# osayamenja/FlashMoE

Hardware: AMD Instinct MI355X
Metric: DMoE fwd tokens/s (higher is better)
Workload: dtype bf16; 1 GPU; BASELINE configs[1]: 1xMI355X E=8 top-2 S=4096 H=1024 P=4096 bf16 (E=8N weak scaling at N ranks); seq_len=4096, d_model=1024, d_ff=4096, experts=8, top_k=2, capacity_factor=1, parallelism=ep1

## Files before the change

### flashmoe_amd/csrc/flashmoe_kernels.hip

```cpp

#include <hip/hip_runtime.h>
#include <hip/hip_bf16.h>
#include <hip/hip_fp16.h>

#include <cmath>
#include <cstdint>
#include <cstdio>
#include <cstring>
#include <algorithm>
#include <type_traits>

#include "../../include/flashmoe_abi.h"


using bf16 = __hip_bfloat16;

struct __align__(8) TPS {
  uint32_t tokenIdx;
  float probSum;
};
__device__ __host__ __forceinline__ uint32_t tpsTok(uint32_t v) {
  return v & 0x0FFFFFFFu;
}
__device__ __host__ __forceinline__ uint32_t tpsJ(uint32_t v) { return v >> 28; }
// ... 242 lines not shown
          if (!tk && lrow[e] > lv) { lv = lrow[e]; li = e; }
        }
#pragma unroll
        for (int off = 1; off < 8; off <<= 1) {
          if (off < SUBS) {
            const float ov = __shfl_xor(lv, off, SUBS);
            const int oi = __shfl_xor(li, off, SUBS);
            if (ov > lv || (ov == lv && oi < li)) { lv = ov; li = oi; }
          }
        }
        if (li >= e0 && li < e1) takenM |= 1ull << (li - e0);
        if (sub == 0) {
          sel[token * K + i] = (uint16_t)li;
          mCw += __expf(lv - m) * inv_d;
        }
      }
      if (sub == 0) sCw[token] = mCw;
    }
  }
  __syncthreads();
  for (int i = tid * 8; i < TT * PX; i += 512 * 8) {
    const int row = i / PX, col0 = i % PX;
    const float mR = sMax[row], ivR = sInv[row];
    const float* lrow = logits + row * (E + 1);
    struct __attribute__((aligned(16))) V8 { T x[8]; } v;
#pragma unroll
    for (int q = 0; q < 8; ++q) {
      const int col = col0 + q;
      const float pv = (col < E) ? __expf(lrow[col] - mR) * ivR : 0.0f;
      fromF(pv, v.x[q]);
    }
    *reinterpret_cast<V8*>(gate_out + (size_t)(pm0 + row) * PX + col0) = v;
  }
  __syncthreads();
  if (tid < E) {
    uint32_t cnt = 0;
    for (int mj = 0; mj < TT * K; mj += 8) {
      const u32x4 v = *reinterpret_cast<const u32x4*>(sel + mj);
#pragma unroll
      for (int q = 0; q < 8; ++q) {
        const uint32_t w = v[q >> 1];
        const uint16_t sv = (q & 1) ? (uint16_t)(w >> 16) : (uint16_t)(w & 0xffff);
        const bool mt = (sv == (uint16_t)tid);
        localIdx[mt ? (mj + q) : TT * K] = (uint16_t)cnt;
        cnt += mt;
      }
    }
    base[tid] = __hip_atomic_fetch_add(eC + tid, cnt, __ATOMIC_RELAXED,
                                       __HIP_MEMORY_SCOPE_AGENT);
    if (gML) {
      float colSum = 0.0f;
      for (int mj = 0; mj < TT; ++mj)
        colSum += __expf(logits[mj * (E + 1) + tid] - sMax[mj]) * sInv[mj];
      atomicAdd(gML + tid, colSum / (float)S);
      atomicAdd(gMeC + tid, (float)cnt / (float)S);
    }
  }
  __syncthreads();
  if (tid < TT) {
#pragma unroll
    for (int i = 0; i < K; ++i) {
      const int e = sel[tid * K + i];
      const uint32_t slot = base[e] + localIdx[tid * K + i];
      const bool keep = slot < (uint32_t)EC;
      if (keep) {
        tokenIds[(size_t)e * pEC + slot] =
            TPS{(uint32_t)(pm0 + tid) | ((uint32_t)i << 28), sCw[tid]};
      }
      if (kept) kept[(size_t)(pm0 + tid) * K + i] = keep ? 1 : 0;
    }
  }
  }
}

template <typename T, int K>
__global__ __launch_bounds__(512) void k_gate_route(
    float* __restrict__ logits32, T* __restrict__ gate_out,
    TPS* __restrict__ tokenIds, uint32_t* __restrict__ eC, int S, int E,
    int PX, int EC, int pEC, float* __restrict__ gML,
    float* __restrict__ gMeC, uint8_t* __restrict__ kept) {
  extern __shared__ __attribute__((aligned(16))) char smem[];
  route_tile_core<T, K>(smem, logits32, gate_out, tokenIds, eC, kept, gML,
                        gMeC, S, E, PX, EC, pEC, blockIdx.x * 128);
}


__device__ __forceinline__ uint32_t cvt2_fp8(float a, float b) {
  f32x2n v;
  v.x = a;
  v.y = b;
  return __builtin_amdgcn_cvt_pk_fp8_f32(v.x, v.y, 0u, false);
}

template <typename T>
__global__ void k_quant_mx(const T* __restrict__ in, uint8_t* __restrict__ out,
                           uint8_t* __restrict__ scales, long long nRows,
                           int K) {
  const int wave = (int)(threadIdx.x >> 6);
  const int lane = (int)(threadIdx.x & 63);
  const long long nBlk = nRows * (K / 64);
  for (long long b = (long long)blockIdx.x * 4 + wave; b < nBlk;
       b += (long long)gridDim.x * 4) {
    const long long row = b / (K / 64);
    const int j = (int)(b % (K / 64));
    const float v = toF(in[row * K + j * 64 + lane]);
    float m = fabsf(v);
#pragma unroll
    for (int off = 32; off > 0; off >>= 1)
      m = fmaxf(m, __shfl_xor(m, off, 64));
    int e = 0;
    if (m > 0.0f) {
      int ex;
      (void)frexpf(m / 448.0f, &ex);
      e = ex;
      if (e < -126) e = -126;
      if (e > 127) e = 127;
    }
    const float inv = exp2f((float)-e);
    const uint32_t pk = cvt2_fp8(v * inv, 0.0f);
    out[row * K + j * 64 + lane] = (uint8_t)(pk & 0xFF);
    if (lane == 0) scales[row * (K / 64) + j] = (uint8_t)(127 + e);
  }
}


struct GemmArgs {
  const void* A;
  const void* B;
  const void* bias;
  void* out;
  float* O32;
  void* moe_out;
  const void* gate_out;
  const TPS* tokenIds;
  const uint32_t* eC;
  long long strideAExpert;
  long long strideBExpert;
  long long strideOExpert;
  int K;
  int N;
  int EC, pEC, PX;
  int topk;
  int act;
  int expertOffset;
  int nRows;
  int H;
  int splitK;
  const int32_t* segExpert;
  int noRemap;
  int totalJobs;
  int jobsMT, jobsNT;
  int atomicLogits;
  int slotAlways;
  int sc1Out;
  const void* aScales;
  void* out8;
  void* outScales;
  long long gluOffset;
};

__device__ __forceinline__ float gate_act(float v, int act) {
  return act == 2 ? v / (1.0f + expf(-v))
                  : 0.5f * v * (1.0f + erff(v * 0.70710678118654752f));
}

typedef __attribute__((address_space(1))) const uint32_t gas_u32;
// ... 1676 lines not shown
      gemm_phase_walk<ET, 0, 256, 128, WET, 3, CH, CP>(
          gu, smem, f.upMT, f.upNT, f.upJobs, f.nBlocks, gu.act,
          gu.bias != nullptr, &f.ctl->upJobsDone, f.upRowDone,
          f.debugBits);
      break;
    default:
      gemm_phase_walk<ET, 0, 128, 128, WET, 2, CH, CP>(
          gu, smem, f.upMT, f.upNT, f.upJobs, f.nBlocks, gu.act,
          gu.bias != nullptr, &f.ctl->upJobsDone, f.upRowDone,
          f.debugBits);
      break;
  }
  if (tid == 0)
    atomicMax(reinterpret_cast<unsigned long long*>(&f.ctl->clk[2]),
              __builtin_amdgcn_s_memrealtime());

  switch (f.dnGeom) {
    case 0:
      gemm_phase_walk_dn<ET, 256, 256, WET, 2, CP, CH>(
          gd, f, smem, f.dnMT, f.dnNT, f.dnJobs, f.nBlocks,
          gd.bias != nullptr, &f.ctl->dnJobsDone);
      break;
    case 1:
      gemm_phase_walk_dn<ET, 128, 256, WET, 3, CP, CH>(
          gd, f, smem, f.dnMT, f.dnNT, f.dnJobs, f.nBlocks,
          gd.bias != nullptr, &f.ctl->dnJobsDone);
      break;
    case 3:
      gemm_phase_walk_dn<ET, 256, 128, WET, 3, CP, CH>(
          gd, f, smem, f.dnMT, f.dnNT, f.dnJobs, f.nBlocks,
          gd.bias != nullptr, &f.ctl->dnJobsDone);
      break;
    default:
      gemm_phase_walk_dn<ET, 128, 128, WET, 2, CP, CH>(
          gd, f, smem, f.dnMT, f.dnNT, f.dnJobs, f.nBlocks,
          gd.bias != nullptr, &f.ctl->dnJobsDone);
      break;
  }
  fused_wait(&f.ctl->dnJobsDone, (uint32_t)f.dnJobs, f.errWord,
             f.spinBound, (f.debugBits & 2) != 0);
  if (tid == 0)
    atomicMax(reinterpret_cast<unsigned long long*>(&f.ctl->clk[3]),
              __builtin_amdgcn_s_memrealtime());

  for (int j = blockIdx.x; j < f.cbJobs; j += f.nBlocks) {
    const int t0 = j * f.cbTB;
    const int t1 = min(f.S, t0 + f.cbTB);
    switch (f.topk) {
      case 1: combine_tokens<ET, 1>(f, t0, t1); break;
      case 2: combine_tokens<ET, 2>(f, t0, t1); break;
      case 3: combine_tokens<ET, 3>(f, t0, t1); break;
      case 4: combine_tokens<ET, 4>(f, t0, t1); break;
      case 5: combine_tokens<ET, 5>(f, t0, t1); break;
      case 6: combine_tokens<ET, 6>(f, t0, t1); break;
      case 7: combine_tokens<ET, 7>(f, t0, t1); break;
      default: combine_tokens<ET, 8>(f, t0, t1); break;
    }
  }
  if (tid == 0)
    atomicMax(reinterpret_cast<unsigned long long*>(&f.ctl->clk[4]),
              __builtin_amdgcn_s_memrealtime());
}


static int launch_group_gemm(hipStream_t st, int phase, const struct GemmArgs& a,
                             int M, int nE);

namespace {

struct State {
  fm_config cfg{};
  bool initialized = false;
  int rank = 0, world = 1;
  int S = 0, H = 0, P = 0, E = 0, PX = 0, nLx = 0, EC = 0, pEC = 0;
  size_t esz = 0;
  size_t wesz = 0;
  int wMats = 2;
  bool gated = false;
  TPS* tokenIds = nullptr;
  uint32_t* eC = nullptr;
  float* logits32 = nullptr;
  float* gML = nullptr;
  float* gMeC = nullptr;
  char* heap = nullptr;
  size_t heapRecvOff = 0, heapRetOff = 0, heapDFlagOff = 0, heapRFlagOff = 0;
  size_t heapBytes = 0;
  void* peerBase[64] = {};
  bool peerOpened[64] = {};
  uint64_t* dPeerRecv = nullptr;
  uint64_t* dPeerRet = nullptr;
  uint64_t* dPeerDFlag = nullptr;
  uint64_t* dPeerRFlag = nullptr;
  uint32_t* dArrive = nullptr;
  uint32_t* hP2pErr = nullptr;
  uint32_t* dP2pErr = nullptr;
  unsigned long long seq = 0;
  hipGraphExec_t graphExec = nullptr;
  void* graphKey[8] = {};
  void* lastKey[8] = {};
  bool graphValid = false;
  void* xM = nullptr;
  uint8_t* x8 = nullptr;
  uint8_t* xs = nullptr;
  uint8_t* xM8 = nullptr;
  uint8_t* xMs = nullptr;
  float* O32 = nullptr;
  void* cbuf = nullptr;
  uint8_t* kept = nullptr;
  int nLxAlloc = 0;
  FusedCtl* fusedCtl = nullptr;
  size_t fusedCtlBytes = 0;
  uint32_t* hFusedErr = nullptr;
  uint32_t* dFusedErr = nullptr;
  int nCU = 0;
  int wallClockKHz = 100000;
  bool lastForwardFused = false;
};
State g;

thread_local char g_err[512] = "";

void setErr(const char* msg) {
  snprintf(g_err, sizeof(g_err), "%s", msg);
}

#define FM_HIP_CHECK(expr)                                                   \
  do {                                                                       \
    hipError_t _e = (expr);                                                  \
    if (_e != hipSuccess) {                                                  \
      snprintf(g_err, sizeof(g_err), "HIP error %s at %s:%d: %s",            \
               hipGetErrorString(_e), __FILE__, __LINE__, #expr);            \
      return FM_ERR_HIP;                                                     \
    }                                                                        \
  } while (0)

static bool mxBigGeom(int M, int N, int nE) {
  return (M >= 256) && (N >= 256) &&
         DIVUP(M, 256) * DIVUP(N, 256) * nE >= (g.nCU > 0 ? g.nCU : 256);
}

static bool mxWideN(int M, int N, int nE) {
  return (N >= 256) &&
         (mxBigGeom(M, N, nE) ||
          DIVUP(M, 128) * DIVUP(N, 256) * nE >= (g.nCU > 0 ? g.nCU : 256));
}

size_t gate_lds_bytes(int E, size_t esz) {
  return 128 * (E + 1) * sizeof(float) + (128 + E) * (64 + 8) * esz;
}

int launch_gate(hipStream_t st, const void* x, const void* gate_w,
                void* gate_out, int64_t S) {
  const int tiles = (int)(S / 128);
  int chunksWanted = DIVUP(512, tiles);
  int Hc = DIVUP(DIVUP(g.H, chunksWanted), 64) * 64;
  const int chunks = DIVUP(g.H, Hc);
  const int eChunks = DIVUP(g.E, 128);
  const int Ec = g.E < 128 ? g.E : 128;
  const bool mfmaLogits = (g.esz == 2);
  const size_t ldsL = gate_lds_bytes(Ec, g.esz);
  const int rTT = (g.E > 256) ? 64 : 128;
  const size_t ldsR = (size_t)rTT * (g.E + 1) * sizeof(float) +
                      rTT * 8 * 2 * sizeof(uint16_t) + g.E * sizeof(uint32_t) +
                      3 * rTT * sizeof(float) + 64;
  float* gMLp = g.cfg.is_training ? g.gML : nullptr;
  float* gMeCp = g.cfg.is_training ? g.gMeC : nullptr;
  if (g.cfg.is_training)
    FM_HIP_CHECK(hipMemsetAsync(g.gML, 0, 2 * (size_t)g.E * sizeof(float), st));
#define GATE_LOGITS(T)                                                        \
  do {                                                                        \
    if (ldsL > 64 * 1024)                                                     \
      (void)hipFuncSetAttribute(reinterpret_cast<const void*>(&k_gate_logits<T>),   \
                          hipFuncAttributeMaxDynamicSharedMemorySize,         \
                          (int)ldsL);                                         \
    hipLaunchKernelGGL((k_gate_logits<T>), dim3(tiles, chunks, eChunks),     \
                       dim3(256), ldsL, st, reinterpret_cast<const T*>(x),    \
                       reinterpret_cast<const T*>(gate_w), g.logits32, g.eC,  \
                       (int)S, g.H, g.E, Hc);                                 \
  } while (0)
#define GATE_ROUTE(T, KK)                                                     \
  do {                                                                        \
    if (ldsR > 64 * 1024)                                                     \
      (void)hipFuncSetAttribute(                                                    \
          reinterpret_cast<const void*>(&k_gate_route<T, KK>),                \
          hipFuncAttributeMaxDynamicSharedMemorySize, (int)ldsR);             \
    hipLaunchKernelGGL((k_gate_route<T, KK>), dim3(tiles), dim3(512), ldsR,   \
                       st, g.logits32, reinterpret_cast<T*>(gate_out),        \
                       g.tokenIds, g.eC, (int)S, g.E, g.PX, g.EC, g.pEC,      \
                       gMLp, gMeCp, g.kept);                                  \
  } while (0)
#define GATE_K(T)                                                             \
  switch (g.cfg.expert_top_k) {                                               \
    case 1: GATE_ROUTE(T, 1); break;                                          \
    case 2: GATE_ROUTE(T, 2); break;                                          \
    case 3: GATE_ROUTE(T, 3); break;                                          \
    case 4: GATE_ROUTE(T, 4); break;                                          \
    case 5: GATE_ROUTE(T, 5); break;                                          \
    case 6: GATE_ROUTE(T, 6); break;                                          \
    case 7: GATE_ROUTE(T, 7); break;                                          \
    case 8: GATE_ROUTE(T, 8); break;                                          \
    default: setErr("unsupported expert_top_k (1..8)"); return FM_ERR_UNSUPPORTED; \
  }
  if (mfmaLogits) {
    GemmArgs ga{};
    ga.A = x;
    ga.B = gate_w;
    ga.out = g.logits32;
    ga.tokenIds = nullptr;
    ga.eC = g.eC;
    ga.EC = g.E;
    ga.K = g.H;
    ga.N = g.E;
    ga.nRows = (int)S;
    ga.H = g.H;
    ga.splitK = 1;
    int rc = launch_group_gemm(st, 3, ga, (int)S, 1);
    if (rc != FM_OK) return rc;
  }
  if (g.cfg.dtype == 2 || g.cfg.dtype == 4 || g.cfg.dtype == 5) {
    if (!mfmaLogits) GATE_LOGITS(bf16);
    GATE_K(bf16)
  } else if (g.cfg.dtype == 3) {
    if (!mfmaLogits) GATE_LOGITS(fp16);
    GATE_K(fp16)
  } else {
    GATE_LOGITS(float);
    GATE_K(float)
  }
#undef GATE_K
#undef GATE_ROUTE
#undef GATE_LOGITS
  FM_HIP_CHECK(hipGetLastError());
  return FM_OK;
}

// ... 274 lines not shown
    return launchFused<bf16, fp8e4m3>(st, gl, gu, gd, f, arena, nBlocks);
  return launchFused<bf16, bf16>(st, gl, gu, gd, f, arena, nBlocks);
}


}

extern "C" {

const char* fm_last_error(void) { return g_err; }
int fm_built_for_gfx950(void) { return 1; }

int fm_initialize(const fm_config* cfg, int rank, int world_size) {
  if (g.initialized) { setErr("already initialized"); return FM_ERR_STATE; }
  if (!cfg) { setErr("null config"); return FM_ERR_STATE; }
  g.cfg = *cfg;
  g.rank = rank;
  g.world = world_size;
  g.S = cfg->sequence_len * cfg->mini_batch;
  g.H = cfg->hidden_size;
  g.P = cfg->intermediate_size;
  g.E = cfg->num_experts;
  g.PX = DIVUP(g.E, 64) * 64;
  if (cfg->num_experts % world_size != 0) {
    setErr("num_experts must divide by world_size (uniform EP split)");
    return FM_ERR_SHAPE;
  }
  g.nLx = g.E / world_size;
  const int base = cfg->drop_tokens ? DIVUP(g.S, g.E) : g.S;
  g.EC = base * cfg->capacity_factor * cfg->expert_top_k;
  g.pEC = DIVUP(g.EC, 128) * 128;
  switch (cfg->dtype) {
    case 0: case 1: g.esz = 4; break;
    case 2: case 3: g.esz = 2; break;
    case 4: g.esz = 2; break;
    case 5: g.esz = 2; break;
    default: setErr("unknown dtype");
             return FM_ERR_UNSUPPORTED;
  }
  g.wesz = (cfg->dtype == 4 || cfg->dtype == 5) ? 1 : g.esz;
  if (cfg->hidden_act < 0 || cfg->hidden_act > 3) {
    setErr("hidden_act must be 0 (relu), 1 (gelu), 2 (swiglu) or 3 (geglu)");
    return FM_ERR_UNSUPPORTED;
  }
  g.gated = cfg->hidden_act >= 2;
  g.wMats = g.gated ? 3 : 2;
  if (g.gated && cfg->dtype == 5) {
    setErr("gated hidden_act (2/3) is not supported with torch_dtype 5 (MX)");
    return FM_ERR_UNSUPPORTED;
  }
  if (cfg->dtype == 5 && (cfg->hidden_size % 128 || cfg->intermediate_size % 128)) {
    setErr("dtype 5 (MX fp8) requires H, P multiples of 128 (BK=128)");
    return FM_ERR_SHAPE;
  }
  if (g.E > 512) { setErr("E > 512 not supported this round"); return FM_ERR_UNSUPPORTED; }
  if (world_size > 64) {
    setErr("world_size > 64 not supported");
    return FM_ERR_UNSUPPORTED;
  }
  if (g.S < 128 || g.S % 128) {
    setErr("S = sequence_len * mini_batch must be a positive multiple of 128");
    return FM_ERR_SHAPE;
  }
  if (cfg->expert_top_k < 1 || cfg->expert_top_k > 8 ||
      cfg->expert_top_k > g.E) {
    setErr("expert_top_k must be in [1, min(E, 8)]");
    return FM_ERR_UNSUPPORTED;
  }
  if (g.H % 64 || g.P % 64) { setErr("H and P must be multiples of 64"); return FM_ERR_SHAPE; }
  g.nLxAlloc = (world_size == 1) ? g.E
                                 : g.nLx * DIVUP(world_size * g.EC, g.pEC);
  FM_HIP_CHECK(hipMalloc(&g.tokenIds, (size_t)g.E * g.pEC * sizeof(TPS)));
  FM_HIP_CHECK(hipMalloc(&g.logits32, (size_t)g.S * g.E * sizeof(float)));
  FM_HIP_CHECK(hipMemset(g.logits32, 0, (size_t)g.S * g.E * sizeof(float)));
  FM_HIP_CHECK(hipMalloc(&g.gML, 2 * (size_t)g.E * sizeof(float)));
  g.gMeC = g.gML + g.E;
  FM_HIP_CHECK(hipMalloc(&g.eC, (size_t)g.E * sizeof(uint32_t)));
  FM_HIP_CHECK(hipMalloc(&g.xM, (size_t)g.nLxAlloc * g.pEC * g.P * g.esz));
  FM_HIP_CHECK(hipMalloc(&g.O32, (size_t)g.S * g.H * sizeof(float)));
  FM_HIP_CHECK(hipMemset(g.O32, 0, (size_t)g.S * g.H * sizeof(float)));
  FM_HIP_CHECK(hipMalloc(&g.cbuf,
                         (size_t)g.S * g.cfg.expert_top_k * g.H * g.esz));
  FM_HIP_CHECK(hipMalloc(&g.kept, (size_t)g.S * g.cfg.expert_top_k));
  if (g.cfg.dtype == 5) {
    const size_t qRows = std::max((size_t)g.S, (size_t)g.nLxAlloc * g.pEC);
    FM_HIP_CHECK(hipMalloc(&g.x8, qRows * g.H));
    FM_HIP_CHECK(hipMalloc(&g.xs, qRows * (g.H / 64)));
    FM_HIP_CHECK(hipMalloc(&g.xM8, (size_t)g.nLxAlloc * g.pEC * g.P));
    FM_HIP_CHECK(hipMalloc(&g.xMs,
                           (size_t)g.nLxAlloc * g.pEC * (g.P / 64)));
  }
  if (g.esz == 2) {
    const int nTiles = g.S / 128;
    g.fusedCtlBytes = sizeof(FusedCtl) + (size_t)nTiles * sizeof(uint32_t) +
                      (size_t)g.E * (g.pEC / 128) * sizeof(uint32_t) +
                      (size_t)g.E * sizeof(uint32_t);
    FM_HIP_CHECK(hipMalloc(&g.fusedCtl, g.fusedCtlBytes));
    FM_HIP_CHECK(hipMemset(g.fusedCtl, 0, g.fusedCtlBytes));
    FM_HIP_CHECK(hipHostMalloc(&g.hFusedErr, sizeof(uint32_t),
                               hipHostMallocMapped));
    *g.hFusedErr = 0;
    FM_HIP_CHECK(hipHostGetDevicePointer(
        reinterpret_cast<void**>(&g.dFusedErr), g.hFusedErr, 0));
    int dev = 0;
    FM_HIP_CHECK(hipGetDevice(&dev));
    int ncu = 0;
    FM_HIP_CHECK(hipDeviceGetAttribute(
        &ncu, hipDeviceAttributeMultiprocessorCount, dev));
    g.nCU = ncu;
    int khz = 0;
    if (hipDeviceGetAttribute(&khz, hipDeviceAttributeWallClockRate, dev) ==
            hipSuccess && khz > 0)
      g.wallClockKHz = khz;
  }
  g.initialized = true;
  return FM_OK;
}

int fm_finalize(void) {
  if (!g.initialized) { setErr("not initialized"); return FM_ERR_STATE; }
  if (g.graphExec) { (void)hipGraphExecDestroy(g.graphExec); g.graphExec = nullptr; }
  (void)hipFree(g.tokenIds); (void)hipFree(g.eC); (void)hipFree(g.xM);
  (void)hipFree(g.O32);
  (void)hipFree(g.cbuf); (void)hipFree(g.kept);
  (void)hipFree(g.logits32); (void)hipFree(g.gML);
  if (g.x8) { (void)hipFree(g.x8); (void)hipFree(g.xs);
              (void)hipFree(g.xM8); (void)hipFree(g.xMs); }
  if (g.fusedCtl) (void)hipFree(g.fusedCtl);
  if (g.hFusedErr) (void)hipHostFree(g.hFusedErr);
  if (g.heap) {
    for (int p = 0; p < g.world; ++p) {
      if (g.peerOpened[p]) (void)hipIpcCloseMemHandle(g.peerBase[p]);
    }
    (void)hipFree(g.heap); (void)hipFree(g.dPeerRecv); (void)hipFree(g.dArrive);
    if (g.hP2pErr) (void)hipHostFree(g.hP2pErr);
  }
  g = State{};
  return FM_OK;
}

int fm_get_compiled_config(int64_t* S, int64_t* H, int64_t* E, int64_t* P,
                           int64_t* PX, int64_t* element_size) {
  if (!g.initialized) { setErr("not initialized"); return FM_ERR_STATE; }
  if (S) *S = g.S;
  if (H) *H = g.H;
  if (E) *E = g.E;
  if (P) *P = g.P;
  if (PX) *PX = g.PX;
  if (element_size) *element_size = (int64_t)g.esz;
  return FM_OK;
}

int fm_get_num_local_experts(void) { return g.initialized ? g.nLx : -1; }

int fm_last_forward_fused(void) {
  return g.initialized ? (g.lastForwardFused ? 1 : 0) : -1;
}

static int launch_group_gemm(hipStream_t st, int phase, const GemmArgs& a,
                             int M, int nE) {
  const int act = (phase == 0) ? a.act : 0;
  const bool gated = act >= 2;
  const bool hasBias = a.bias != nullptr;
  if (gated && hasBias) {
    setErr("b_up is not supported with a gated hidden_act (2/3)");
    return FM_ERR_UNSUPPORTED;
  }
  const int N = gated ? 2 * a.N : a.N;
  const long long gluOffset = gated ? 2LL * a.N * a.K : 0;
  if (g.cfg.dtype == 5 && phase != 3) {
    GemmArgs aa = a;
    aa.splitK = 1;
    aa.totalJobs = 0;
    static const int forceBig = [] {
      const char* e2 = getenv("FM_MX_GEOM");
      return (e2 && e2[0] == 'b') ? 1 : 0;
    }();
    const bool big = forceBig && mxBigGeom(M, N, nE);
    const bool mid = !big && (N >= 256) &&
                     DIVUP(M, 128) * DIVUP(N, 256) * nE >=
                         (g.nCU > 0 ? g.nCU : 256);
    const int bm = big ? 256 : 128, bn = (big || mid) ? 256 : 128;
    static const bool mxS3 = [] {
      const char* e2 = getenv("FM_MX_STAGES");
      return !(e2 && e2[0] == '2');
    }();
    dim3 grid(DIVUP(M, bm), DIVUP(N, bn), nE);
    dim3 block(512);
    {
      const int J = grid.x * grid.y * nE;
      const int resident = (big ? 1 : 2) * (g.nCU > 0 ? g.nCU : 256);
      if (J > resident) {
        aa.totalJobs = J;
        aa.jobsMT = grid.x;
        aa.jobsNT = grid.y;
        grid = dim3(resident, 1, 1);
      }
    }
#define MXGG(PH, AC, HB)                                                      \
    do {                                                                      \
      if (big)                                                                \
        hipLaunchKernelGGL((k_group_gemm_mx<PH, AC, HB, 256, 256>), grid,     \
                           block, 0, st, aa);                                 \
      else if (mid && mxS3)                                                   \
        hipLaunchKernelGGL((k_group_gemm_mx<PH, AC, HB, 128, 256, 3>), grid,  \
                           block, 0, st, aa);                                 \
      else if (mid)                                                           \
        hipLaunchKernelGGL((k_group_gemm_mx<PH, AC, HB, 128, 256>), grid,     \
// ... 276 lines not shown
  if (evs) FM_HIP_CHECK(hipEventRecord(evs[1], st));

  int rc = launch_gate(st, x, gate_w, gate_out, S);
  if (rc != FM_OK) return rc;
  if (evs) FM_HIP_CHECK(hipEventRecord(evs[2], st));

  if (g.cfg.dtype == 5) {
    rc = launch_quant_mx(st, x, g.x8, g.xs, g.S, g.H);
    if (rc != FM_OK) return rc;
  }

  GemmArgs up{};
  up.A = (g.cfg.dtype == 5) ? (const void*)g.x8 : x;
  up.aScales = g.xs;
  up.B = expert_w;
  up.bias = b_up;
  up.out = g.xM;
  up.gate_out = gate_out;
  up.tokenIds = g.tokenIds;
  up.eC = g.eC;
  up.strideAExpert = 0;
  up.strideBExpert = (long long)g.wMats * g.P * g.H;
  up.strideOExpert = (long long)g.pEC * g.P;
  up.K = g.H; up.N = g.P;
  up.EC = g.EC; up.pEC = g.pEC; up.PX = g.PX;
  up.topk = g.cfg.expert_top_k; up.act = g.cfg.hidden_act;
  up.expertOffset = 0; up.nRows = 0; up.H = g.H;
  const bool mxEpiQuant =
      (g.cfg.dtype == 5) && mxWideN(g.pEC, g.P, g.E);
  if (mxEpiQuant) {
    up.out8 = g.xM8;
    up.outScales = g.xMs;
  }
  rc = launch_group_gemm(st, 0, up, g.pEC, g.E);
  if (rc != FM_OK) return rc;
  if (evs) FM_HIP_CHECK(hipEventRecord(evs[3], st));

  if (g.cfg.dtype == 5 && !mxEpiQuant) {
    rc = launch_quant_mx(st, g.xM, g.xM8, g.xMs,
                         (long long)g.E * g.pEC, g.P);
    if (rc != FM_OK) return rc;
  }

  GemmArgs dn = up;
  dn.out8 = nullptr;
  dn.outScales = nullptr;
  dn.A = (g.cfg.dtype == 5) ? (const void*)g.xM8 : g.xM;
  dn.aScales = g.xMs;
  dn.B = reinterpret_cast<const char*>(expert_w) + (size_t)g.P * g.H * g.wesz;
  dn.bias = b_dn;
  dn.out = nullptr;
  dn.O32 = reinterpret_cast<float*>(g.cbuf);
  dn.moe_out = moe_out;
  dn.strideAExpert = (long long)g.pEC * g.P;
  dn.K = g.P; dn.N = g.H;
  rc = launch_group_gemm(st, 1, dn, g.pEC, g.E);
  if (rc != FM_OK) return rc;
  if (evs) FM_HIP_CHECK(hipEventRecord(evs[4], st));

  if (g.cfg.expert_top_k > 1) {
    int rc2 = launch_cast_combine(st, moe_out);
    if (rc2 != FM_OK) return rc2;
  }
  return FM_OK;
}

int fm_moe_forward(void* stream, const void* x, const void* gate_w,
                   const void* expert_w, const void* b_up, const void* b_dn,
                   void* gate_out, void* moe_out, int64_t S) {
  if (!g.initialized) { setErr("not initialized"); return FM_ERR_STATE; }
  if (g.world != 1) {
    setErr("fm_moe_forward is the single-rank path; use the staged EP entry points");
    return FM_ERR_STATE;
  }
  if (S != g.S) { setErr("S mismatch vs frozen config"); return FM_ERR_SHAPE; }
  int prc = fusedPoisonCheck();
  if (prc != FM_OK) return prc;
  hipStream_t st = reinterpret_cast<hipStream_t>(stream);

  void* key[8] = {const_cast<void*>(x), const_cast<void*>(gate_w),
                  const_cast<void*>(expert_w), const_cast<void*>(b_up),
                  const_cast<void*>(b_dn), gate_out, moe_out,
                  reinterpret_cast<void*>(static_cast<uintptr_t>(
                      (uint64_t)S << 1 | (fusedEnabled() ? 1 : 0)))};
  if (g.graphValid && memcmp(key, g.graphKey, sizeof(key)) == 0) {
    if (hipGraphLaunch(g.graphExec, st) == hipSuccess) return FM_OK;
    g.graphValid = false;
  }
  if (st != nullptr && memcmp(key, g.lastKey, sizeof(key)) == 0) {
    if (g.graphExec) { (void)hipGraphExecDestroy(g.graphExec); g.graphExec = nullptr; }
    if (hipStreamBeginCapture(st, hipStreamCaptureModeThreadLocal) ==
        hipSuccess) {
      int rc = moe_forward_impl(st, x, gate_w, expert_w, b_up, b_dn, gate_out,
                                moe_out, S, nullptr);
      hipGraph_t graph = nullptr;
      hipError_t ec = hipStreamEndCapture(st, &graph);
      if (rc == FM_OK && ec == hipSuccess && graph) {
        if (hipGraphInstantiate(&g.graphExec, graph, nullptr, nullptr, 0) ==
            hipSuccess) {
          memcpy(g.graphKey, key, sizeof(key));
          g.graphValid = true;
          (void)hipGraphDestroy(graph);
          if (hipGraphLaunch(g.graphExec, st) == hipSuccess) return FM_OK;
          g.graphValid = false;
        } else {
          (void)hipGraphDestroy(graph);
        }
      } else if (graph) {
        (void)hipGraphDestroy(graph);
      }
      if (rc != FM_OK) return rc;
    }
  }
  memcpy(g.lastKey, key, sizeof(key));
  return moe_forward_impl(st, x, gate_w, expert_w, b_up, b_dn, gate_out,
                          moe_out, S, nullptr);
}

int fm_moe_forward_phased(void* stream, const void* x, const void* gate_w,
                          const void* expert_w, const void* b_up,
                          const void* b_dn, void* gate_out, void* moe_out,
                          int64_t S, float ms[4]) {
  if (!g.initialized) { setErr("not initialized"); return FM_ERR_STATE; }
  if (g.world != 1) { setErr("single-rank path only"); return FM_ERR_STATE; }
  if (S != g.S) { setErr("S mismatch vs frozen config"); return FM_ERR_SHAPE; }
  hipStream_t st = reinterpret_cast<hipStream_t>(stream);
  hipEvent_t evs[6];
  for (auto& e : evs) FM_HIP_CHECK(hipEventCreate(&e));
  FM_HIP_CHECK(hipEventRecord(evs[0], st));
  int rc = moe_forward_impl(st, x, gate_w, expert_w, b_up, b_dn, gate_out,
                            moe_out, S, evs);
  if (rc == FM_OK) {
    FM_HIP_CHECK(hipEventRecord(evs[5], st));
    FM_HIP_CHECK(hipStreamSynchronize(st));
    if (g.lastForwardFused) {
      int prc = fusedPoisonCheck();
      if (prc != FM_OK) { rc = prc; }
      else {
        FusedCtl hc;
        FM_HIP_CHECK(hipMemcpy(&hc, g.fusedCtl, sizeof(hc),
                               hipMemcpyDeviceToHost));
        const double khz = (double)g.wallClockKHz;
        ms[0] = (float)((double)(hc.clk[1] - hc.clk[0]) / khz);
        ms[1] = (float)((double)(hc.clk[2] - hc.clk[1]) / khz);
        ms[2] = (float)((double)(hc.clk[3] - hc.clk[2]) / khz);
        ms[3] = (float)((double)(hc.clk[4] - hc.clk[3]) / khz);
      }
    } else {
      float pre = 0, gate = 0, upT = 0, dnT = 0, post = 0;
      (void)hipEventElapsedTime(&pre, evs[0], evs[1]);
      (void)hipEventElapsedTime(&gate, evs[1], evs[2]);
      (void)hipEventElapsedTime(&upT, evs[2], evs[3]);
      (void)hipEventElapsedTime(&dnT, evs[3], evs[4]);
      (void)hipEventElapsedTime(&post, evs[4], evs[5]);
      ms[0] = gate; ms[1] = upT; ms[2] = dnT; ms[3] = pre + post;
    }
  }
  for (auto& e : evs) (void)hipEventDestroy(e);
  return rc;
}

int fm_gate_forward(void* stream, const void* x, const void* gate_w,
                    void* gate_out, int64_t S) {
  if (!g.initialized) { setErr("not initialized"); return FM_ERR_STATE; }
  if (S != g.S) { setErr("S mismatch vs frozen config"); return FM_ERR_SHAPE; }
  hipStream_t st = reinterpret_cast<hipStream_t>(stream);
  return launch_gate(st, x, gate_w, gate_out, S);
// ... 555 lines not shown
```

Measured before the change: 24.94 million tokens/s.

## Fuse gate logits, softmax, top-k and routing into a single kernel

Adds a gate kernel that computes gate logits with MFMA, then softmax, top-k selection and gate output in one launch. Each block handles 16 tokens, and the last block to finish a 128-token tile uses atomic arrival counters to assign slots for the whole tile. This replaces the separate logits and routing launches, along with the fp32 logits round-trip through global memory. The cost is atomic counters and a cross-block completion protocol that has to reset itself for graph replay. It applies only to 16-bit, inference mode with E<=64, and can be turned off with an environment variable.

```diff
diff --git a/flashmoe_amd/csrc/flashmoe_kernels.hip b/flashmoe_amd/csrc/flashmoe_kernels.hip
--- a/flashmoe_amd/csrc/flashmoe_kernels.hip
+++ b/flashmoe_amd/csrc/flashmoe_kernels.hip
@@ -348,6 +348,248 @@
   extern __shared__ __attribute__((aligned(16))) char smem[];
   route_tile_core<T, K>(smem, logits32, gate_out, tokenIds, eC, kept, gML,
                         gMeC, S, E, PX, EC, pEC, blockIdx.x * 128);
+}
+
+
+__device__ __forceinline__ uint32_t gate_arrive(uint32_t* ctr,
+                                                uint32_t lastVal,
+                                                uint32_t* sFlag) {
+  asm volatile("s_waitcnt vmcnt(0)" ::: "memory");
+  __syncthreads();
+  if (threadIdx.x == 0) {
+    const uint32_t old = __hip_atomic_fetch_add(ctr, 1u, __ATOMIC_RELAXED,
+                                                __HIP_MEMORY_SCOPE_AGENT);
+    if (old == lastVal) __builtin_amdgcn_fence(__ATOMIC_ACQUIRE, "agent");
+    *sFlag = old;
+  }
+  __syncthreads();
+  return *sFlag;
+}
+
+template <typename T, int NE, int U>
+__device__ __forceinline__ void gate_logits_trip(const T* __restrict__ xrow,
+                                                 const T* const (&wp)[NE],
+                                                 int s, f32x4 (&acc)[4]) {
+  using vec8 = typename ETr<T>::vec8;
+  vec8 xv[U], wv[U][NE];
+#pragma unroll
+  for (int u = 0; u < U; ++u) {
+    xv[u] = *reinterpret_cast<const vec8*>(xrow + (s + u) * 32);
+#pragma unroll
+    for (int f = 0; f < NE; ++f)
+      wv[u][f] = *reinterpret_cast<const vec8*>(wp[f] + (s + u) * 32);
+  }
+#pragma unroll
+  for (int u = 0; u < U; ++u)
+#pragma unroll
+    for (int f = 0; f < NE; ++f)
+      acc[f] = ETr<T>::mfma(wv[u][f], xv[u], acc[f]);
+}
+
+template <typename T, int NE>
+__device__ __forceinline__ void gate_logits_wave(const T* __restrict__ xrow,
+                                                 const T* __restrict__ gate_w,
+                                                 int H, int E, int lane,
+                                                 int s0, int s1,
+                                                 f32x4 (&acc)[4]) {
+  const T* wp[NE];
+#pragma unroll
+  for (int f = 0; f < NE; ++f)
+    wp[f] = gate_w + (size_t)min(f * 16 + (lane & 15), E - 1) * H +
+            (lane >> 4) * 8;
+  int s = s0;
+  for (; s + 8 <= s1; s += 8) gate_logits_trip<T, NE, 8>(xrow, wp, s, acc);
+  if (s + 4 <= s1) { gate_logits_trip<T, NE, 4>(xrow, wp, s, acc); s += 4; }
+  for (; s < s1; ++s) gate_logits_trip<T, NE, 1>(xrow, wp, s, acc);
+}
+
+template <typename T, int K, int TB>
+__global__ __launch_bounds__(TB * 16) void k_gate_fused(
+    const T* __restrict__ x, const T* __restrict__ gate_w,
+    T* __restrict__ gate_out, uint16_t* gateSel, float* gateCw,
+    uint32_t* tilesDone, uint32_t* tileArrive, uint32_t* eCacc,
+    TPS* __restrict__ tokenIds, uint32_t* __restrict__ eC,
+    uint8_t* __restrict__ kept, int H, int E, int PX, int EC, int pEC) {
+  constexpr int NT = TB * 16;
+  constexpr int NWV = NT / 64;
+  constexpr int SUB = 128 / TB;
+  constexpr int LDP = 68;
+  constexpr int LDL = 65;
+  __shared__ __attribute__((aligned(16))) float part[NWV * 16 * LDP];
+  __shared__ float logits[TB * LDL];
+  __shared__ float sInv[TB], sMax[TB];
+  __shared__ __attribute__((aligned(16))) uint16_t sSel[128 * K];
+  __shared__ uint16_t sLoc[128 * K];
+  __shared__ float sCw[128];
+  __shared__ uint32_t cntH[2 * 64];
+  __shared__ uint32_t base[64];
+  __shared__ uint32_t sFlag[2];
+
+  const int tid = threadIdx.x;
+  const int wave = tid >> 6, lane = tid & 63;
+  const int tile = blockIdx.x / SUB;
+  const int m0 = blockIdx.x * TB;
+
+  {
+    const int kSteps = H / 32;
+    const int spw = DIVUP(kSteps, 4);
+    const int ks = wave & 3, rg = wave >> 2;
+    const int s0 = min(ks * spw, kSteps);
+    const int s1 = min(s0 + spw, kSteps);
+    f32x4 acc[4];
+#pragma unroll
+    for (int f = 0; f < 4; ++f) acc[f] = f32x4{0.f, 0.f, 0.f, 0.f};
+    const T* xrow =
+        x + (size_t)(m0 + rg * 16 + (lane & 15)) * H + (lane >> 4) * 8;
+    const int NEr = DIVUP(E, 16);
+    if (NEr == 1) gate_logits_wave<T, 1>(xrow, gate_w, H, E, lane, s0, s1, acc);
+    else if (NEr == 2) gate_logits_wave<T, 2>(xrow, gate_w, H, E, lane, s0, s1, acc);
+    else gate_logits_wave<T, 4>(xrow, gate_w, H, E, lane, s0, s1, acc);
+    float* prow = part + (wave * 16 + (lane & 15)) * LDP + (lane >> 4) * 4;
+#pragma unroll
+    for (int f = 0; f < 4; ++f)
+      if (f < NEr) *reinterpret_cast<f32x4*>(prow + f * 16) = acc[f];
+  }
+  __syncthreads();
+  for (int i = tid; i < TB * E; i += NT) {
+    const int row = i / E, col = i % E;
+    const float* p = part + ((row >> 4) * 4 * 16 + (row & 15)) * LDP + col;
+    float v = p[0];
+    v += p[16 * LDP];
+    v += p[2 * 16 * LDP];
+    v += p[3 * 16 * LDP];
+    logits[row * LDL + col] = v;
+  }
+  __syncthreads();
+
+  if (tid < TB * 4) {
+    constexpr int SUBS = 4;
+    const int token = tid / SUBS;
+    const int sub = tid % SUBS;
+    const float* lrow = logits + token * LDL;
+    const int chunk = (E + SUBS - 1) / SUBS;
+    const int e0 = min(E, sub * chunk);
+    const int e1 = min(E, e0 + chunk);
+    float m = -INFINITY;
+    for (int e = e0; e < e1; ++e) m = fmaxf(m, lrow[e]);
+#pragma unroll
+    for (int off = 1; off < SUBS; off <<= 1)
+      m = fmaxf(m, __shfl_xor(m, off, SUBS));
+    float d = 0.0f;
+    for (int e = e0; e < e1; ++e) d += __expf(lrow[e] - m);
+#pragma unroll
+    for (int off = 1; off < SUBS; off <<= 1) d += __shfl_xor(d, off, SUBS);
+    const float inv_d = 1.0f / d;
+    if (sub == 0) {
+      sInv[token] = inv_d;
+      sMax[token] = m;
+    }
+    uint32_t takenM = 0u;
+    float mCw = 0.0f;
+#pragma unroll
+    for (int i = 0; i < K; ++i) {
+      float lv = -INFINITY;
+      int li = E;
+      for (int e = e0; e < e1; ++e) {
+        const bool tk = (takenM >> (e - e0)) & 1u;
+        if (!tk && lrow[e] > lv) { lv = lrow[e]; li = e; }
+      }
+#pragma unroll
+      for (int off = 1; off < SUBS; off <<= 1) {
+        const float ov = __shfl_xor(lv, off, SUBS);
+        const int oi = __shfl_xor(li, off, SUBS);
+        if (ov > lv || (ov == lv && oi < li)) { lv = ov; li = oi; }
+      }
+      if (li >= e0 && li < e1) takenM |= 1u << (li - e0);
+      if (sub == 0) {
+        __hip_atomic_store(gateSel + (size_t)(m0 + token) * K + i,
+                           (uint16_t)li, __ATOMIC_RELAXED,
+                           __HIP_MEMORY_SCOPE_AGENT);
+        mCw += __expf(lv - m) * inv_d;
+      }
+    }
+    if (sub == 0)
+      __hip_atomic_store(gateCw + m0 + token, mCw, __ATOMIC_RELAXED,
+                         __HIP_MEMORY_SCOPE_AGENT);
+  }
+  const bool lastOfTile =
+      gate_arrive(tileArrive + tile, SUB - 1, &sFlag[0]) == SUB - 1;
+  for (int i = tid * 8; i < TB * PX; i += NT * 8) {
+    const int row = i / PX, col0 = i % PX;
+    const float mR = sMax[row], ivR = sInv[row];
+    const float* lrow = logits + row * LDL;
+    struct __attribute__((aligned(16))) V8 { T x[8]; } v;
+#pragma unroll
+    for (int q = 0; q < 8; ++q) {
+      const int col = col0 + q;
+      const float pv = (col < E) ? __expf(lrow[col] - mR) * ivR : 0.0f;
+      fromF(pv, v.x[q]);
+    }
+    *reinterpret_cast<V8*>(gate_out + (size_t)(m0 + row) * PX + col0) = v;
+  }
+
+  if (!lastOfTile) return;
+
+  const int t0 = tile * 128;
+  for (int i = tid; i < 128 * K; i += NT)
+    sSel[i] = __hip_atomic_load(gateSel + (size_t)t0 * K + i, __ATOMIC_RELAXED,
+                                __HIP_MEMORY_SCOPE_AGENT);
+  for (int i = tid; i < 128; i += NT)
+    sCw[i] = __hip_atomic_load(gateCw + t0 + i, __ATOMIC_RELAXED,
+                               __HIP_MEMORY_SCOPE_AGENT);
+  __syncthreads();
+  {
+    const int half = wave & 1;
+    const int tok = half * 64 + lane;
+    uint16_t s[K];
+#pragma unroll
+    for (int j = 0; j < K; ++j) s[j] = sSel[tok * K + j];
+    for (int e = wave >> 1; e < E; e += NWV / 2) {
+      int hj = -1;
+#pragma unroll
+      for (int j = 0; j < K; ++j)
+        if (s[j] == (uint16_t)e) hj = j;
+      const unsigned long long mk = __ballot(hj >= 0);
+      const uint32_t pre = __builtin_amdgcn_mbcnt_hi(
+          (uint32_t)(mk >> 32), __builtin_amdgcn_mbcnt_lo((uint32_t)mk, 0u));
+      if (hj >= 0) sLoc[tok * K + hj] = (uint16_t)pre;
+      if (lane == 0) cntH[half * 64 + e] = (uint32_t)__popcll(mk);
+    }
+  }
+  __syncthreads();
+  if (tid < E)
+    base[tid] = __hip_atomic_fetch_add(eCacc + tid, cntH[tid] + cntH[64 + tid],
+                                       __ATOMIC_RELAXED,
+                                       __HIP_MEMORY_SCOPE_AGENT);
+  const uint32_t nTiles = gridDim.x / SUB;
+  if (gate_arrive(tilesDone, nTiles - 1, &sFlag[1]) == nTiles - 1) {
+    if (tid < E) {
+      eC[tid] = __hip_atomic_load(eCacc + tid, __ATOMIC_RELAXED,
+                                  __HIP_MEMORY_SCOPE_AGENT);
+      __hip_atomic_store(eCacc + tid, 0u, __ATOMIC_RELAXED,
+                         __HIP_MEMORY_SCOPE_AGENT);
+    }
+    if (tid == 0)
+      __hip_atomic_store(tilesDone, 0u, __ATOMIC_RELAXED,
+                         __HIP_MEMORY_SCOPE_AGENT);
+  }
+  if (tid == 0)
+    __hip_atomic_store(tileArrive + tile, 0u, __ATOMIC_RELAXED,
+                       __HIP_MEMORY_SCOPE_AGENT);
+  for (int i = tid; i < 128 * K; i += NT) {
+    const int tok = i / K, j = i % K;
+    const int e = sSel[i];
+    bool keep = false;
+    if (e < E) {
+      const uint32_t slot =
+          base[e] + sLoc[i] + (tok >= 64 ? cntH[e] : 0u);
+      keep = slot < (uint32_t)EC;
+      if (keep)
+        tokenIds[(size_t)e * pEC + slot] =
+            TPS{(uint32_t)(t0 + tok) | ((uint32_t)j << 28), sCw[tok]};
+    }
+    if (kept) kept[(size_t)(t0 + tok) * K + j] = keep ? 1 : 0;
+  }
 }
 
 
@@ -2190,6 +2432,8 @@
   float* logits32 = nullptr;
   float* gML = nullptr;
   float* gMeC = nullptr;
+  uint32_t* gateCtl = nullptr;
+  size_t gateArriveOff = 0, gateEcOff = 0, gateCwOff = 0, gateSelOff = 0;
   char* heap = nullptr;
   size_t heapRecvOff = 0, heapRetOff = 0, heapDFlagOff = 0, heapRFlagOff = 0;
   size_t heapBytes = 0;
@@ -2257,8 +2501,55 @@
   return 128 * (E + 1) * sizeof(float) + (128 + E) * (64 + 8) * esz;
 }
 
+static bool gateFusedEnabled() {
+  const char* e = getenv("FM_GATE_FUSED");
+  return !(e && e[0] == '0');
+}
+
+static bool gateFusedApplies() {
+  return g.gateCtl && g.esz == 2 && g.E <= 64 && !g.cfg.is_training &&
+         gateFusedEnabled();
+}
+
+constexpr int kGateTB = 16;
+
+template <typename T>
+int launch_gate_fused(hipStream_t st, const void* x, const void* gate_w,
+                      void* gate_out, int64_t S) {
+  char* ws = reinterpret_cast<char*>(g.gateCtl);
+#define GATE_FUSED(KK)                                                        \
+  hipLaunchKernelGGL((k_gate_fused<T, KK, kGateTB>),                          \
+                     dim3((unsigned)(S / kGateTB)), dim3(kGateTB * 16), 0,    \
+                     st, reinterpret_cast<const T*>(x),                       \
+                     reinterpret_cast<const T*>(gate_w),                      \
+                     reinterpret_cast<T*>(gate_out),                          \
+                     reinterpret_cast<uint16_t*>(ws + g.gateSelOff),          \
+                     reinterpret_cast<float*>(ws + g.gateCwOff), g.gateCtl,   \
+                     reinterpret_cast<uint32_t*>(ws + g.gateArriveOff),       \
+                     reinterpret_cast<uint32_t*>(ws + g.gateEcOff),           \
+                     g.tokenIds, g.eC, g.kept, g.H, g.E, g.PX, g.EC, g.pEC)
+  switch (g.cfg.expert_top_k) {
+    case 1: GATE_FUSED(1); break;
+    case 2: GATE_FUSED(2); break;
+    case 3: GATE_FUSED(3); break;
+    case 4: GATE_FUSED(4); break;
+    case 5: GATE_FUSED(5); break;
+    case 6: GATE_FUSED(6); break;
+    case 7: GATE_FUSED(7); break;
+    case 8: GATE_FUSED(8); break;
+    default: setErr("unsupported expert_top_k (1..8)"); return FM_ERR_UNSUPPORTED;
+  }
+#undef GATE_FUSED
+  FM_HIP_CHECK(hipGetLastError());
+  return FM_OK;
+}
+
 int launch_gate(hipStream_t st, const void* x, const void* gate_w,
                 void* gate_out, int64_t S) {
+  if (gateFusedApplies())
+    return g.cfg.dtype == 3
+               ? launch_gate_fused<fp16>(st, x, gate_w, gate_out, S)
+               : launch_gate_fused<bf16>(st, x, gate_w, gate_out, S);
   const int tiles = (int)(S / 128);
   int chunksWanted = DIVUP(512, tiles);
   int Hc = DIVUP(DIVUP(g.H, chunksWanted), 64) * 64;
@@ -2699,6 +2990,18 @@
   FM_HIP_CHECK(hipMalloc(&g.cbuf,
                          (size_t)g.S * g.cfg.expert_top_k * g.H * g.esz));
   FM_HIP_CHECK(hipMalloc(&g.kept, (size_t)g.S * g.cfg.expert_top_k));
+  if (g.esz == 2 && g.E <= 64 && !g.cfg.is_training) {
+    auto up16 = [](size_t v) { return (v + 15) & ~(size_t)15; };
+    g.gateArriveOff = 16;
+    g.gateEcOff = g.gateArriveOff + up16((size_t)(g.S / 128) * sizeof(uint32_t));
+    g.gateCwOff = g.gateEcOff + up16((size_t)g.E * sizeof(uint32_t));
+    g.gateSelOff = g.gateCwOff + up16((size_t)g.S * sizeof(float));
+    const size_t bytes =
+        g.gateSelOff +
+        up16((size_t)g.S * g.cfg.expert_top_k * sizeof(uint16_t));
+    FM_HIP_CHECK(hipMalloc(&g.gateCtl, bytes));
+    FM_HIP_CHECK(hipMemset(g.gateCtl, 0, bytes));
+  }
   if (g.cfg.dtype == 5) {
     const size_t qRows = std::max((size_t)g.S, (size_t)g.nLxAlloc * g.pEC);
     FM_HIP_CHECK(hipMalloc(&g.x8, qRows * g.H));
@@ -2741,6 +3044,7 @@
   (void)hipFree(g.O32);
   (void)hipFree(g.cbuf); (void)hipFree(g.kept);
   (void)hipFree(g.logits32); (void)hipFree(g.gML);
+  if (g.gateCtl) (void)hipFree(g.gateCtl);
   if (g.x8) { (void)hipFree(g.x8); (void)hipFree(g.xs);
               (void)hipFree(g.xM8); (void)hipFree(g.xMs); }
   if (g.fusedCtl) (void)hipFree(g.fusedCtl);
@@ -3183,7 +3487,8 @@
                   const_cast<void*>(expert_w), const_cast<void*>(b_up),
                   const_cast<void*>(b_dn), gate_out, moe_out,
                   reinterpret_cast<void*>(static_cast<uintptr_t>(
-                      (uint64_t)S << 1 | (fusedEnabled() ? 1 : 0)))};
+                      (uint64_t)S << 2 | (gateFusedEnabled() ? 2 : 0) |
+                      (fusedEnabled() ? 1 : 0)))};
   if (g.graphValid && memcmp(key, g.graphKey, sizeof(key)) == 0) {
     if (hipGraphLaunch(g.graphExec, st) == hipSuccess) return FM_OK;
     g.graphValid = false;
```

Result: faster. 26.43 million tokens/s, median of 6 (+6.0%).
